# rrwick/Polypolish

Hardware: NVIDIA H100
Metric: assembly Mbp polished/sec (higher is better)
Workload: dtype u8 bases / u32 counters / f64 depth

## Files before the change

### polypolish_b200/csrc/polish_dev.cuh

```cuda
#pragma once

#include "nib_utils.h"
#include "../../include/pp_abi.h"

#define PP_BIN_SHIFT 8
#define PP_BIN (1u << PP_BIN_SHIFT)
#define PP_SUB_SHIFT 7
#define PP_SUB (1u << PP_SUB_SHIFT)
#define TL_T 2048
#define TL_THREADS 512
#define TL_PER_THREAD (TL_T / TL_THREADS)
#define TL_LONG_E 512
#define TL_QCAP 1024
#define TL_FAST_LEN 192
#define PR_THREADS 256
#define SC_GROUP_SCAN_LIMIT 8192
#define VT_THREADS 256
#define VT_ITEMS 8
#define VT_CHUNK (VT_THREADS * VT_ITEMS)
#define NONE32 0xFFFFFFFFu
static_assert(VT_CHUNK == TL_T, "k_tile hands k_compact one chunk per tile");
static_assert(TL_T % PP_BIN == 0 && TL_T / PP_SUB == TL_THREADS / 32 && TL_PER_THREAD * 32 == PP_SUB, "tile = whole bins; warp w owns depth sub-tile w and votes on it");

enum : unsigned {
// ... 1515 lines not shown
#endif
        __syncthreads();
        if (tid == 0) {
            long long t = 0;
            for (int i = 0; i < TL_THREADS / 32; ++i) t += sh.s_delta[i];
            vp.chunk_delta[tile] = t;
#ifdef PP_TILE_PROF
            pt[5] = clock64();
            for (int i = 0; i < 5; ++i) atomicAdd(&d.st->prof[i], (unsigned long long)(pt[i + 1] - pt[i]));
            atomicAdd(&d.st->prof[5], (unsigned long long)sh.qn);
            atomicAdd(&d.st->prof[6], 1ull);
            atomicMax(&d.st->prof[7], (unsigned long long)sh.qn);
#endif
        }
    }
}
static_assert(TL_PER_THREAD == 4, "the verdict store packs four positions per thread");

#if !defined(PP_EMULATE)
template <int BITS, bool CHG>
__global__ void __launch_bounds__(TL_THREADS, 1) k_tile(DevData d, VoteParams vp) {
    extern __shared__ __align__(16) unsigned char tile_smem[];
    tile_body<BITS, CHG>(d, vp, *reinterpret_cast<TileShared*>(tile_smem));
}
#endif

__device__ __forceinline__ uint8_t* put_u32(uint8_t* w, uint32_t v) {
    w[0] = (uint8_t)v; w[1] = (uint8_t)(v >> 8); w[2] = (uint8_t)(v >> 16); w[3] = (uint8_t)(v >> 24);
    return w + 4;
}
template <int BITS>
__device__ void allele_strings_row(const OthCtx& oc, uint32_t pos, uint32_t new_node, uint8_t* pool, unsigned long long cap,
                                   unsigned long long* used, unsigned long long* off) {
    unsigned long long bytes = 8;
    uint32_t n = 0;
    for (uint32_t nd = oc.head[pos]; nd != 0; nd = oc.nodes[nd - 1].next == NONE32 ? 0 : oc.nodes[nd - 1].next + 1) {
        bytes += 8 + ((uint32_t)oc.nodes[nd - 1].val & 0xFFFFu);
        n++;
    }
    const uint32_t new_len = new_node == NONE32 ? 0u : (uint32_t)oc.nodes[new_node].val & 0xFFFFu;
    bytes += new_len;
    const unsigned long long o = atomicAdd(used, bytes);
    *off = o;
    if (o + bytes > cap) return;
    uint8_t* w = put_u32(pool + o, n);
    for (uint32_t nd = oc.head[pos]; nd != 0; nd = oc.nodes[nd - 1].next == NONE32 ? 0 : oc.nodes[nd - 1].next + 1) {
        const uint32_t len = (uint32_t)oc.nodes[nd - 1].val & 0xFFFFu;
        w = put_u32(put_u32(w, oc.nodes[nd - 1].count), len);
        for (uint32_t t = 0; t < len; ++t) *w++ = other_char<BITS>(oc, nd - 1, t);
    }
    w = put_u32(w, new_len);
    for (uint32_t t = 0; t < new_len; ++t) *w++ = other_char<BITS>(oc, new_node, t);
}
template <int BITS>
__device__ void allele_strings_body(const OthCtx& oc, const uint32_t* pos, const pp_debug_pos* rec, bool by_pos, uint32_t n, uint8_t* pool,
                                    unsigned long long cap, unsigned long long* used, unsigned long long* off) {
    for (uint32_t i = blockIdx.x * blockDim.x + threadIdx.x; i < n; i += gridDim.x * blockDim.x) {
        const uint32_t p = pos[i];
        allele_strings_row<BITS>(oc, p, rec[by_pos ? p : i].new_node, pool, cap, used, off + i);
    }
}
#if !defined(PP_EMULATE)
template <int BITS>
__global__ void __launch_bounds__(256) k_allele_strings(OthCtx oc, const uint32_t* pos, const pp_debug_pos* rec, bool by_pos, uint32_t n,
                                                         uint8_t* pool, unsigned long long cap, unsigned long long* used, unsigned long long* off) {
    allele_strings_body<BITS>(oc, pos, rec, by_pos, n, pool, cap, used, off);
}
#endif

#define CP_STAGE (VT_CHUNK + 2048)
struct CompactShared {
    unsigned long long s_warp[VT_THREADS / 32];
    unsigned long long s_total;
    long long s_red[VT_THREADS / 32];
    long long s_base;
    __align__(16) uint8_t s_out[CP_STAGE];
};

template <int BITS>
__device__ __forceinline__ void compact_body(const DevData& d, const VoteParams& vp, CompactShared& sh) {
    const uint32_t tid = threadIdx.x, chunk = blockIdx.x;
    const uint32_t p0 = chunk * VT_CHUNK + tid * VT_ITEMS;
    long long acc = 0;
    for (uint32_t j = tid; j < chunk; j += VT_THREADS) acc += vp.chunk_delta[j];
    for (int o = 16; o > 0; o >>= 1) acc += __shfl_down_sync(0xffffffffu, acc, o);
    if ((tid & 31) == 0) sh.s_red[tid >> 5] = acc;
    __syncthreads();
    if (tid == 0) {
        long long t = 0;
        for (int i = 0; i < VT_THREADS / 32; ++i) t += sh.s_red[i];
        sh.s_base = (long long)chunk * VT_CHUNK + t;
    }
    const uint4 rv = *reinterpret_cast<const uint4*>(vp.res + p0);
    const uint32_t w[4] = {rv.x, rv.y, rv.z, rv.w};
    uint32_t len[VT_ITEMS];
    unsigned long long tlen = 0;
    OthCtx oc;
    oc.nodes = d.nodes; oc.head = d.oth_head;
    oc.sr = SeqRef{d.seq_pool, d.seq_off, d.seq_len, d.flags};
#pragma unroll
    for (int i = 0; i < VT_ITEMS; ++i) {
        const uint32_t h = (w[i >> 1] >> ((i & 1) * 16)) & 0xFFFFu;
        uint32_t l = h >> 8;
        if (p0 + i >= d.G) l = 0;
        else if (l == 255) {
            const uint32_t rec = vp.rec_at[p0 + i];
            const uint32_t rlen = (uint32_t)oc.nodes[rec].val & 0xFFFFu;
            l = 0;
            for (uint32_t t = 0; t < rlen; ++t) l += other_char<BITS>(oc, rec, t) != '-';
        }
        len[i] = l;
        tlen += l;
    }
    const unsigned long long oexcl = block_exscan<VT_THREADS>(tlen, sh.s_warp, &sh.s_total);
    const unsigned long long total = sh.s_total;
    const unsigned long long base = (unsigned long long)sh.s_base;
    if (chunk == vp.n_chunks - 1 && tid == 0) { vp.out_off[d.n_contigs] = base + total; d.st->out_len = base + total; }
    if (p0 < d.G) {
        uint32_t lo = 0, hi = d.n_contigs;
        while (lo < hi) { const uint32_t mid = (lo + hi) >> 1; if (d.contig_off[mid] < p0) lo = mid + 1; else hi = mid; }
        if (lo < d.n_contigs && d.contig_off[lo] < (unsigned long long)p0 + VT_ITEMS) {
            unsigned long long oo = base + oexcl;
            uint32_t c = lo;
#pragma unroll
            for (int i = 0; i < VT_ITEMS; ++i) {
                while (c < d.n_contigs && d.contig_off[c] == p0 + i) { vp.out_off[c] = oo; c++; }
                oo += len[i];
            }
        }
    }
    if (base + total > vp.out_cap) { if (tid == 0) atomicOr(&d.st->flags, (unsigned)FL_OUT_OVF); return; }
    const bool staged = total <= CP_STAGE;
    uint8_t* dst = staged ? sh.s_out : vp.out + base;
    unsigned long long o = oexcl;
#pragma unroll
    for (int i = 0; i < VT_ITEMS; ++i) {
        if (len[i] == 0) continue;
        const uint32_t h = (w[i >> 1] >> ((i & 1) * 16)) & 0xFFFFu;
        if ((h >> 8) != 255) { dst[o++] = (uint8_t)h; continue; }
        const uint32_t rec = vp.rec_at[p0 + i];
        const uint32_t rlen = (uint32_t)oc.nodes[rec].val & 0xFFFFu;
        for (uint32_t t = 0; t < rlen; ++t) {
            const uint8_t ch = other_char<BITS>(oc, rec, t);
            if (ch != '-') dst[o++] = ch;
        }
    }
    if (!staged) return;
    __syncthreads();
    uint8_t* g = vp.out + base;
    const uint32_t n = (uint32_t)total;
    const uint32_t head = min(n, (uint32_t)((16 - ((size_t)g & 15)) & 15));
    for (uint32_t i = tid; i < head; i += VT_THREADS) g[i] = sh.s_out[i];
    const uint32_t nvec = (n - head) / 16;
    for (uint32_t i = tid; i < nvec; i += VT_THREADS) {
        const uint8_t* sp = sh.s_out + head + i * 16;
        uint32_t x[4];
#pragma unroll
        for (int k = 0; k < 4; ++k) x[k] = sp[4 * k] | (sp[4 * k + 1] << 8) | (sp[4 * k + 2] << 16) | ((uint32_t)sp[4 * k + 3] << 24);
        reinterpret_cast<uint4*>(g + head)[i] = make_uint4(x[0], x[1], x[2], x[3]);
    }
    for (uint32_t i = head + nvec * 16 + tid; i < n; i += VT_THREADS) g[i] = sh.s_out[i];
}

#if !defined(PP_EMULATE)
template <int BITS>
__global__ void __launch_bounds__(VT_THREADS) k_compact(DevData d, VoteParams vp) {
    __shared__ CompactShared sh;
    compact_body<BITS>(d, vp, sh);
}
#endif
```

### polypolish_b200/csrc/polish_kernels.cu

```cuda
#include <cuda_runtime.h>

#include <cub/device/device_radix_sort.cuh>
#include <cub/device/device_scan.cuh>

#include <algorithm>
#include <functional>
#include <cstddef>
#include <cstdio>
#include <string>
#include <vector>

#include "pp_internal.h"
#include "pp_ctx.cuh"
#include "polish_dev.cuh"


static void init_comp_table(uint8_t* t) {
    for (int i = 0; i < 256; ++i) t[i] = 'N';
    const char* a = "ATGCNRYSWKMBVDH.-?";
    const char* b = "TACGNYRSWMKVBHD.-?";
    for (int i = 0; a[i]; ++i) t[(unsigned char)a[i]] = (uint8_t)b[i];
}

extern "C" const char* pp_version(void) { return "0.6.1-b200"; }

extern "C" void* pp_host_alloc(size_t bytes) {
    void* p = nullptr;
    if (cudaHostAlloc(&p, bytes ? bytes : 1, cudaHostAllocDefault) != cudaSuccess) { cudaGetLastError(); return nullptr; }
    return p;
}
extern "C" void pp_host_free(void* p) { if (p) cudaFreeHost(p); }

#define PP_INIT_IMAGE (64u << 10)

extern "C" int pp_create(int device, pp_ctx** out) {
    if (!out) return PP_ERR_ARG;
    *out = nullptr;
    int n = 0;
    cudaError_t e = cudaGetDeviceCount(&n);
    if (e != cudaSuccess || n == 0 || device < 0 || device >= n) { cudaGetLastError(); return PP_ERR_CUDA; }
    pp_ctx* ctx = new pp_ctx();
    ctx->device = device;
    if (cudaSetDevice(device) != cudaSuccess) { delete ctx; return PP_ERR_CUDA; }
    cudaDeviceProp prop;
    if (cudaGetDeviceProperties(&prop, device) != cudaSuccess || prop.major != 9 || prop.minor != 0) { delete ctx; return PP_ERR_CUDA; }
    ctx->sm_count = prop.multiProcessorCount;
    if (cudaStreamCreateWithFlags(&ctx->stream, cudaStreamNonBlocking) != cudaSuccess) { delete ctx; return PP_ERR_CUDA; }
    if (cudaStreamCreateWithFlags(&ctx->copy_stream, cudaStreamNonBlocking) != cudaSuccess) { delete ctx; return PP_ERR_CUDA; }
    if (cudaEventCreateWithFlags(&ctx->ev_small, cudaEventDisableTiming) != cudaSuccess ||
        cudaEventCreateWithFlags(&ctx->ev_seq, cudaEventDisableTiming) != cudaSuccess) { delete ctx; return PP_ERR_CUDA; }
    for (auto& ev : ctx->ev) if (cudaEventCreate(&ev) != cudaSuccess) { delete ctx; return PP_ERR_CUDA; }
    if (cudaHostAlloc((void**)&ctx->h_status, sizeof(DevStatus), cudaHostAllocDefault) != cudaSuccess) { delete ctx; return PP_ERR_CUDA; }
    if (cudaHostAlloc((void**)&ctx->h_params, sizeof(DevParams), cudaHostAllocDefault) != cudaSuccess) { delete ctx; return PP_ERR_CUDA; }
    if (cudaHostAlloc((void**)&ctx->h_init, PP_INIT_IMAGE, cudaHostAllocDefault) != cudaSuccess) { delete ctx; return PP_ERR_CUDA; }
    uint8_t comp[256];
    init_comp_table(comp);
    if (cudaMemcpyToSymbol(c_comp, comp, 256) != cudaSuccess) { delete ctx; return PP_ERR_CUDA; }
    *out = ctx;
    return PP_OK;
}

extern "C" void pp_destroy(pp_ctx* ctx) {
    if (!ctx) return;
    cudaSetDevice(ctx->device);
    if (ctx->stream) cudaStreamSynchronize(ctx->stream);
    pp_tok_release(ctx);
    for (auto& b : ctx->b) b.release();
    for (auto& ev : ctx->ev) if (ev) cudaEventDestroy(ev);
    if (ctx->h_status) cudaFreeHost(ctx->h_status);
    if (ctx->h_params) cudaFreeHost(ctx->h_params);
    if (ctx->h_init) cudaFreeHost(ctx->h_init);
    if (ctx->ev_small) cudaEventDestroy(ctx->ev_small);
    if (ctx->ev_seq) cudaEventDestroy(ctx->ev_seq);
    if (ctx->copy_stream) cudaStreamDestroy(ctx->copy_stream);
    if (ctx->stream) cudaStreamDestroy(ctx->stream);
    delete ctx;
}

extern "C" const char* pp_last_error(const pp_ctx* ctx) { return ctx ? ctx->err.c_str() : "null context"; }

int pp_ctx_fail(pp_ctx* ctx, int code, const char* msg) { ctx->err = msg; return code; }
int pp_ctx_device(pp_ctx* ctx) { return ctx->device; }
int pp_ctx_sm_count(pp_ctx* ctx) { return ctx->sm_count; }
cudaStream_t pp_ctx_stream(pp_ctx* ctx) { return ctx->stream; }
cudaEvent_t pp_ctx_event(pp_ctx* ctx, int i) { return ctx->ev[i]; }
void pp_ctx_count_launches(pp_ctx* ctx, uint32_t n) { ctx->launches = n; }
int pp_ctx_fail_cuda(pp_ctx* ctx, cudaError_t e, const char* what, const char* file, int line) {
    ctx->err = std::string("CUDA error: ") + cudaGetErrorString(e) + " at " + what + " (" + file + ":" + std::to_string(line) + ")";
    return PP_ERR_CUDA;
}
void* pp_ctx_scratch2(pp_ctx* ctx, size_t bytes) {
    if (ctx->b[B_SCRATCH2].ensure(bytes) != cudaSuccess) { cudaGetLastError(); return nullptr; }
    return ctx->b[B_SCRATCH2].p;
}
void* pp_ctx_scratch(pp_ctx* ctx, size_t bytes) {
    if (ctx->b[B_SCRATCH].ensure(bytes) != cudaSuccess) { cudaGetLastError(); return nullptr; }
    return ctx->b[B_SCRATCH].p;
}

template <class T>
static int upload(pp_ctx* ctx, int which, const T* src, size_t n, size_t pad_bytes = 64) {
    CK(ctx->b[which].ensure(n * sizeof(T) + pad_bytes));
    if (n) CK(cudaMemcpyAsync(ctx->b[which].p, src, n * sizeof(T), cudaMemcpyHostToDevice, ctx->stream));
    return PP_OK;
}

int pp_ctx_upload_contigs(pp_ctx* ctx, const pp_contigs* c) {
    if (!c || !c->off || !c->bases || c->n_contigs == 0) return ctx->fail(PP_ERR_ARG, "null or empty contigs");
    const uint64_t G = c->off[c->n_contigs];
    if (G == 0 || G >= 0xFFFFFFFFull - 2 * VT_CHUNK) return ctx->fail(PP_ERR_ARG, "total assembly length must be in [1, 2^32-4096)");
    int rc;
    if ((rc = upload(ctx, B_DRAFT, c->bases, G, VT_CHUNK + 256))) return rc;
    if ((rc = upload(ctx, B_CTGOFF, c->off, (size_t)c->n_contigs + 1))) return rc;
    ctx->G = G; ctx->n_contigs = c->n_contigs;
    return PP_OK;
}

static void fill_data(pp_ctx* ctx, DevData& d) {
    const uint64_t G = ctx->G;
    memset(&d, 0, sizeof d);
    d.n_aln = ctx->n_aln;
    d.contig = ctx->b[B_CONTIG].as<uint32_t>(); d.ref_start = ctx->b[B_REFSTART].as<uint32_t>();
    d.read_id = ctx->b[B_READID].as<uint32_t>(); d.seq_off = ctx->b[B_SEQOFF].as<uint32_t>();
    d.cigar_off = ctx->b[B_CIGOFF].as<uint32_t>(); d.nm = ctx->b[B_NM].as<uint32_t>();
    d.cigar_ops = ctx->b[B_CIGOPS].as<uint32_t>(); d.seq_len = ctx->b[B_SEQLEN].as<uint16_t>();
    d.n_cigar = ctx->b[B_NCIG].as<uint16_t>(); d.flags = ctx->b[B_FLAGS].as<uint8_t>();
    d.seq_pool = ctx->b[B_SEQPOOL].as<uint8_t>(); d.draft = ctx->b[B_DRAFT].as<uint8_t>();
    d.contig_off = ctx->b[B_CTGOFF].as<unsigned long long>(); d.n_contigs = ctx->n_contigs; d.G = (uint32_t)G;
    d.n_bins = (uint32_t)((G + PP_BIN - 1) >> PP_BIN_SHIFT); d.n_tiles = (uint32_t)((G + TL_T - 1) / TL_T);
    d.recs = ctx->b[B_RECS].as<TileRec>(); d.key = ctx->b[B_KEY].as<uint32_t>(); d.val = ctx->b[B_VAL].as<uint32_t>();
    d.sval = ctx->b[B_SVAL].as<uint32_t>(); d.bin_start = ctx->b[B_BINSTART].as<uint32_t>();
    d.srec = ctx->b[B_SREC].as<TileRec>(); d.sseq = ctx->b[B_SSEQ].as<uint4>();
    d.n_slots = ctx->n_slots; d.max_ext = ctx->max_ext;
    d.tile_order = ctx->b[B_TILEORDER].as<uint32_t>();
    d.kf = ctx->b[B_KF].as<uint32_t>(); d.wrec = ctx->b[B_NK].as<uint4>(); d.errc = ctx->b[B_ERRC].as<uint8_t>(); d.gq = ctx->b[B_GQ].as<uint16_t>();
}

template <int BITS>
static int bin_dataset(pp_ctx* ctx, const std::function<int()>& seq_ready) {
    cudaStream_t s = ctx->stream;
    const uint64_t n_aln = ctx->n_aln, G = ctx->G;
    const uint32_t n_bins = (uint32_t)((G + PP_BIN - 1) >> PP_BIN_SHIFT);
    int key_bits = 1;
    while ((1ull << key_bits) < (uint64_t)n_bins + 2) key_bits++;
    const size_t na = (size_t)n_aln + 16;
    CK(ctx->b[B_RECS].ensure(na * sizeof(TileRec)));
    CK(ctx->b[B_KEY].ensure(na * 4)); CK(ctx->b[B_VAL].ensure(na * 4));
    CK(ctx->b[B_SKEY].ensure(na * 4)); CK(ctx->b[B_SVAL].ensure(na * 4));
    CK(ctx->b[B_BINSTART].ensure(((size_t)n_bins + 4) * 4));
// ... 163 lines not shown
    const uint64_t seq_bytes = two_bit ? n_blocks2 * 16 + a->esc_pool_bytes : a->seq_pool_bytes;
    CK(ctx->b[B_SEQPOOL].ensure(seq_bytes + 256));
    if (two_bit) CK(ctx->b[B_SEQ2].ensure(a->seq_pool_bytes + 256));
    CK(cudaEventRecord(ctx->ev_small, ctx->stream));
    CK(cudaStreamWaitEvent(ctx->copy_stream, ctx->ev_small, 0));
    if (!two_bit) {
        if (a->seq_pool_bytes) CK(cudaMemcpyAsync(ctx->b[B_SEQPOOL].p, a->seq_pool, a->seq_pool_bytes, cudaMemcpyHostToDevice, ctx->copy_stream));
    } else {
        if (a->seq_pool_bytes) CK(cudaMemcpyAsync(ctx->b[B_SEQ2].p, a->seq_pool, a->seq_pool_bytes, cudaMemcpyHostToDevice, ctx->copy_stream));
        if (a->esc_pool_bytes)
            CK(cudaMemcpyAsync(ctx->b[B_SEQPOOL].as<uint8_t>() + n_blocks2 * 16, a->esc_pool, a->esc_pool_bytes, cudaMemcpyHostToDevice, ctx->copy_stream));
        if (a->esc_pool_bytes && a->n_aln)
            k_esc_offsets<<<(uint32_t)std::min<uint64_t>((a->n_aln + 255) / 256, (uint64_t)ctx->sm_count * 32), 256, 0, ctx->stream>>>(
                ctx->b[B_SEQOFF].as<uint32_t>(), ctx->b[B_FLAGS].as<uint8_t>(), a->n_aln, (uint32_t)n_blocks2);
    }
    CK(cudaEventRecord(ctx->ev_seq, ctx->copy_stream));
    auto seq_ready = [&]() -> int {
        CK(cudaStreamWaitEvent(ctx->stream, ctx->ev_seq, 0));
        if (two_bit && n_blocks2)
            k_expand2<<<(uint32_t)std::min<uint64_t>((n_blocks2 + 255) / 256, (uint64_t)ctx->sm_count * 32), 256, 0, ctx->stream>>>(
                ctx->b[B_SEQ2].as<uint2>(), ctx->b[B_SEQPOOL].as<uint4>(), n_blocks2);
        return PP_OK;
    };
    rc = commit_dataset(ctx, a->n_aln, a->n_reads, a->n_cigar_ops, seq_bytes, two_bit ? 4u : a->seq_bits, seq_ready);
    if (rc != PP_OK) cudaStreamSynchronize(ctx->copy_stream);
    return rc;
}

static const char* err_text(unsigned code) {
    switch (code) {
        case ERR_UNKNOWN_CONTIG: return "query name in SAM but not in assembly";
        case ERR_SEQ_MISMATCH: return "CIGAR string does not match read sequence";
        case ERR_BAD_OP: return "unexpected character (other than M, =, X, I or D) in CIGAR string - did you use BWA MEM to generate your alignments?";
        case ERR_OOB: return "alignment extends past the end of its reference sequence";
        case ERR_NOSEQ: return "no alignments for read contain sequence";
        default: return "unknown device-side error";
    }
}

template <int BITS>
static int run_polish(pp_ctx* ctx, const pp_polish_params* prm, pp_polish_result* res) {
    cudaStream_t s = ctx->stream;
    const uint64_t G = ctx->G, n_aln = ctx->n_aln;
    const uint32_t n_tiles = (uint32_t)((G + TL_T - 1) / TL_T);
    const size_t padG = (size_t)n_tiles * TL_T + 16;
    ctx->have_changes = false;

    CK(ctx->b[B_OUTOFF].ensure(((size_t)ctx->n_contigs + 1) * 8));
    CK(ctx->b[B_RES].ensure(padG * 2)); CK(ctx->b[B_RECAT].ensure((G + 1) * 4)); CK(ctx->b[B_CHUNKDELTA].ensure((size_t)n_tiles * 8));
    CK(ctx->b[B_PARAMS].ensure(sizeof(DevParams)));
    if (!ctx->tile_attr_set) {
        CK(cudaFuncSetAttribute(k_tile<4, false>, cudaFuncAttributeMaxDynamicSharedMemorySize, (int)sizeof(TileShared)));
        CK(cudaFuncSetAttribute(k_tile<8, false>, cudaFuncAttributeMaxDynamicSharedMemorySize, (int)sizeof(TileShared)));
        CK(cudaFuncSetAttribute(k_tile<4, true>, cudaFuncAttributeMaxDynamicSharedMemorySize, (int)sizeof(TileShared)));
        CK(cudaFuncSetAttribute(k_tile<8, true>, cudaFuncAttributeMaxDynamicSharedMemorySize, (int)sizeof(TileShared)));
        ctx->tile_attr_set = true;
    }

    ctx->h_params->fv = prm->fraction_valid; ctx->h_params->fi = prm->fraction_invalid;
    ctx->h_params->min_depth = prm->min_depth; ctx->h_params->max_errors = prm->max_errors;
    ctx->h_params->careful = prm->careful ? 1 : 0; ctx->h_params->pad = 0;

    for (int attempt = 0; attempt < 8; ++attempt) {
        const uint32_t node_cap = ctx->node_cap;
        const uint64_t out_cap = ctx->out_cap;
        size_t zoff = 0;
        auto carve = [&](size_t bytes) { size_t o = zoff; zoff += (bytes + 255) & ~size_t(255); return o; };
        const size_t o_chg = carve((size_t)ctx->n_contigs * 8), o_zero = carve((size_t)ctx->n_contigs * 8),
                     o_tdep = carve((size_t)ctx->n_contigs * 8), o_status = carve(sizeof(DevStatus)),
                     o_k = carve(ctx->global_k ? (ctx->n_reads + 1) * 4 : 4), o_prm = carve(sizeof(DevParams));
        const bool one_copy = zoff <= PP_INIT_IMAGE;
        CK(ctx->b[B_ZEROPOOL].ensure(zoff));
        CK(ctx->b[B_HEADS].ensure(padG * 4 + 64));
        uint8_t* zp = ctx->b[B_ZEROPOOL].as<uint8_t>();
        CK(ctx->b[B_NODES].ensure((size_t)node_cap * sizeof(OthNode)));
        CK(ctx->b[B_OUT].ensure(out_cap + 64));

        DevData d;
        fill_data(ctx, d);
        d.k = (uint32_t*)(zp + o_k);
        d.oth_head = ctx->b[B_HEADS].as<uint32_t>(); d.nodes = ctx->b[B_NODES].as<OthNode>(); d.node_cap = node_cap;
        d.prm = one_copy ? (DevParams*)(zp + o_prm) : ctx->b[B_PARAMS].as<DevParams>();
        d.st = (DevStatus*)(zp + o_status);
        ctx->launches = 0;

        CK(cudaEventRecord(ctx->ev[0], s));
        if (one_copy) {
            memset(ctx->h_init, 0, zoff);
            memcpy(ctx->h_init + o_prm, ctx->h_params, sizeof(DevParams));
            memset(ctx->h_init + o_status + offsetof(DevStatus, err), 0xFF, 8);
            CK(cudaMemcpyAsync(zp, ctx->h_init, zoff, cudaMemcpyHostToDevice, s));
        } else {
            CK(cudaMemcpyAsync(ctx->b[B_PARAMS].p, ctx->h_params, sizeof(DevParams), cudaMemcpyHostToDevice, s));
            CK(cudaMemsetAsync(zp, 0, zoff, s));
            CK(cudaMemsetAsync(&d.st->err, 0xFF, 8, s));
        }
        CK(cudaEventRecord(ctx->ev[1], s));
        if (n_aln && ctx->global_k) {
            k_classify_multi<<<(uint32_t)std::min<uint64_t>((n_aln + 255) / 256, (uint64_t)ctx->sm_count * 8), 256, 0, s>>>(d);
            ctx->launches++;
        }
        CK(cudaEventRecord(ctx->ev[2], s));
        if (n_aln) {
            const uint32_t grid = (uint32_t)std::min<uint64_t>((n_aln + PR_THREADS - 1) / PR_THREADS, (uint64_t)ctx->sm_count * 8);
            if (ctx->global_k) k_goodk<true><<<grid, PR_THREADS, 0, s>>>(d);
            else k_goodk<false><<<grid, PR_THREADS, 0, s>>>(d);
            ctx->launches++;
        }
        CK(cudaEventRecord(ctx->ev[3], s));
        VoteParams vp;
        vp.n_chunks = n_tiles;
        vp.out = ctx->b[B_OUT].as<uint8_t>(); vp.out_cap = out_cap;
        vp.out_off = ctx->b[B_OUTOFF].as<unsigned long long>();
        vp.changed = (unsigned long long*)(zp + o_chg); vp.zero_depth = (unsigned long long*)(zp + o_zero); vp.total_depth = (double*)(zp + o_tdep);
        vp.res = ctx->b[B_RES].as<uint16_t>(); vp.rec_at = ctx->b[B_RECAT].as<uint32_t>();
        vp.chunk_delta = ctx->b[B_CHUNKDELTA].as<long long>();
        vp.dbg = nullptr;
        if (ctx->debug_on) { CK(ctx->b[B_DEBUG].ensure((G + 1) * sizeof(pp_debug_pos))); vp.dbg = ctx->b[B_DEBUG].as<pp_debug_pos>(); }
        vp.chg = nullptr; vp.chg_pos = nullptr; vp.chg_n = &d.st->n_changes; vp.chg_cap = 0;
        if (ctx->changes_on) {
            if (ctx->chg_cap == 0) ctx->chg_cap = (uint32_t)std::max<uint64_t>(4096, G / 256);
            CK(ctx->b[B_CHG].ensure((size_t)ctx->chg_cap * sizeof(pp_debug_pos))); CK(ctx->b[B_CHGPOS].ensure((size_t)ctx->chg_cap * 4));
            vp.chg = ctx->b[B_CHG].as<pp_debug_pos>(); vp.chg_pos = ctx->b[B_CHGPOS].as<uint32_t>(); vp.chg_cap = ctx->chg_cap;
        }
        {
            int occ = 1;
            CK(cudaOccupancyMaxActiveBlocksPerMultiprocessor(&occ, vp.chg ? k_tile<BITS, true> : k_tile<BITS, false>, TL_THREADS, sizeof(TileShared)));
            const uint32_t grid = std::min<uint32_t>(n_tiles, (uint32_t)ctx->sm_count * (uint32_t)std::max(occ, 1));
            if (vp.chg) k_tile<BITS, true><<<grid, TL_THREADS, sizeof(TileShared), s>>>(d, vp);
            else k_tile<BITS, false><<<grid, TL_THREADS, sizeof(TileShared), s>>>(d, vp);
            ctx->launches++;
        }
        CK(cudaEventRecord(ctx->ev[4], s));
        k_compact<BITS><<<n_tiles, VT_THREADS, 0, s>>>(d, vp);
        ctx->launches++;
        CK(cudaEventRecord(ctx->ev[5], s));
        CK(cudaMemcpyAsync(ctx->h_status, d.st, sizeof(DevStatus), cudaMemcpyDeviceToHost, s));
        CK(cudaStreamSynchronize(s));
        CK(cudaGetLastError());
        const DevStatus hs = *ctx->h_status;
#ifdef PP_TILE_PROF
        fprintf(stderr, "[tile prof] tiles %llu; cycles/tile: A %.0f B %.0f queue %.0f C %.0f D+E %.0f; queued reads/tile %.1f (max %llu); "
                "chunk wait/tile/warp %.0f\n", hs.prof[6],
                (double)hs.prof[0] / hs.prof[6], (double)hs.prof[1] / hs.prof[6], (double)hs.prof[2] / hs.prof[6], (double)hs.prof[3] / hs.prof[6],
                (double)hs.prof[4] / hs.prof[6], (double)hs.prof[5] / hs.prof[6], hs.prof[7], (double)hs.prof[11] / hs.prof[6] / (TL_THREADS / 32));
        fprintf(stderr, "[tile prof] depth walks %llu (%.2f per tile, %llu tiles with one), %.0f cycles each\n", hs.prof[9], (double)hs.prof[9] / hs.prof[6], hs.prof[10],
                hs.prof[9] ? (double)hs.prof[8] / hs.prof[9] : 0.0);
#endif
        if (hs.err != ~0ull) {
            res->error_aln = (int64_t)(hs.err >> 8);
            return ctx->fail(PP_ERR_INPUT, std::string(err_text((unsigned)(hs.err & 0xFF))) + " (alignment " + std::to_string(hs.err >> 8) + ")");
        }
        bool again = false;
        if (hs.flags & FL_BIGGROUP) { if (ctx->global_k) return ctx->fail(PP_ERR_CUDA, "internal error: FL_BIGGROUP in global-k mode"); ctx->global_k = true; again = true; }
        if (hs.flags & FL_NODE_OVF) { ctx->node_cap = (uint32_t)std::min<uint64_t>(0x7FFFFFFFull, (uint64_t)hs.node_count + hs.node_count / 4 + 1024); again = true; }
        if (!again && (hs.flags & FL_OUT_OVF)) { ctx->out_cap = hs.out_len + 64; again = true; }
        if (!again && ctx->changes_on && hs.n_changes > ctx->chg_cap) { ctx->chg_cap = hs.n_changes; again = true; }
        if (again) continue;

        ctx->have_debug = ctx->debug_on; ctx->last_head = d.oth_head; ctx->last_nodes = std::min(hs.node_count, node_cap);
        ctx->have_changes = ctx->changes_on; ctx->n_changes = ctx->changes_on ? hs.n_changes : 0; ctx->chg_pool = -1;
        res->out_len = hs.out_len;
        res->n_aln_used = hs.n_used;
        res->error_aln = -1;
        memset(&res->timing, 0, sizeof res->timing);
        float ms;
        CK(cudaEventElapsedTime(&ms, ctx->ev[0], ctx->ev[1])); res->timing.stage_ms[0] = ms;
        CK(cudaEventElapsedTime(&ms, ctx->ev[1], ctx->ev[2])); res->timing.stage_ms[1] = ms;
        CK(cudaEventElapsedTime(&ms, ctx->ev[2], ctx->ev[3])); res->timing.stage_ms[2] = ms;
        CK(cudaEventElapsedTime(&ms, ctx->ev[3], ctx->ev[4])); res->timing.stage_ms[3] = ms;
        CK(cudaEventElapsedTime(&ms, ctx->ev[4], ctx->ev[5])); res->timing.stage_ms[4] = ms;
        CK(cudaEventElapsedTime(&ms, ctx->ev[0], ctx->ev[5])); res->timing.total_ms = ms;
        res->timing.launches = ctx->launches;

        if (res->out_bases) {
            if (res->out_cap < hs.out_len) return ctx->fail(PP_ERR_ARG, "out_cap too small: need " + std::to_string(hs.out_len) + " bytes");
            CK(cudaEventRecord(ctx->ev[7], s));
            CK(cudaMemcpyAsync(res->out_bases, vp.out, hs.out_len, cudaMemcpyDeviceToHost, s));
            if (res->out_off) CK(cudaMemcpyAsync(res->out_off, vp.out_off, ((size_t)ctx->n_contigs + 1) * 8, cudaMemcpyDeviceToHost, s));
            if (res->changed) CK(cudaMemcpyAsync(res->changed, vp.changed, (size_t)ctx->n_contigs * 8, cudaMemcpyDeviceToHost, s));
            if (res->zero_depth) CK(cudaMemcpyAsync(res->zero_depth, vp.zero_depth, (size_t)ctx->n_contigs * 8, cudaMemcpyDeviceToHost, s));
            if (res->total_depth) CK(cudaMemcpyAsync(res->total_depth, vp.total_depth, (size_t)ctx->n_contigs * 8, cudaMemcpyDeviceToHost, s));
            CK(cudaEventRecord(ctx->ev[8], s));
            CK(cudaStreamSynchronize(s));
            CK(cudaEventElapsedTime(&ms, ctx->ev[7], ctx->ev[8]));
            res->timing.stage_ms[7] = ms;
        }
        return PP_OK;
    }
    return ctx->fail(PP_ERR_NOMEM, "side buffers kept overflowing");
}

static int check_params(pp_ctx* ctx, const pp_polish_params* p) {
    if (!p) return ctx->fail(PP_ERR_ARG, "null params");
    if (!(p->fraction_valid > 0.0 && p->fraction_valid < 1.0)) return ctx->fail(PP_ERR_INPUT, "--fraction_valid must be between 0 and 1 (exclusive)");
    if (!(p->fraction_invalid > 0.0 && p->fraction_invalid < 1.0)) return ctx->fail(PP_ERR_INPUT, "--fraction_invalid must be between 0 and 1 (exclusive)");
    if (p->fraction_invalid >= p->fraction_valid) return ctx->fail(PP_ERR_INPUT, "--fraction_invalid must be less than --fraction_valid");
    return PP_OK;
}

extern "C" int pp_polish_resident(pp_ctx* ctx, const pp_polish_params* params, pp_polish_result* result) {
    if (!ctx) return PP_ERR_ARG;
    if (!result) return ctx->fail(PP_ERR_ARG, "null result");
    if (!ctx->have_ds) return ctx->fail(PP_ERR_ARG, "pp_polish_resident: no dataset uploaded");
    int rc = check_params(ctx, params);
    if (rc) return rc;
    CK(cudaSetDevice(ctx->device));
    result->error_aln = -1;
    return ctx->seq_bits == 4 ? run_polish<4>(ctx, params, result) : run_polish<8>(ctx, params, result);
}

extern "C" int pp_polish(pp_ctx* ctx, const pp_contigs* contigs, const pp_alignments* alns,
                         const pp_polish_params* params, pp_polish_result* result) {
    if (!ctx) return PP_ERR_ARG;
    if (!result) return ctx->fail(PP_ERR_ARG, "null result");
    int rc = check_params(ctx, params);
    if (rc) return rc;
    CK(cudaSetDevice(ctx->device));
    CK(cudaEventRecord(ctx->ev[9], ctx->stream));
    rc = pp_dataset_upload(ctx, contigs, alns);
    if (rc) return rc;
    CK(cudaEventRecord(ctx->ev[10], ctx->stream));
    CK(cudaEventSynchronize(ctx->ev[10]));
    float h2d = 0;
    CK(cudaEventElapsedTime(&h2d, ctx->ev[9], ctx->ev[10]));
    result->error_aln = -1;
    rc = ctx->seq_bits == 4 ? run_polish<4>(ctx, params, result) : run_polish<8>(ctx, params, result);
    if (rc == PP_OK) result->timing.stage_ms[6] = h2d;
    return rc;
}

extern "C" int pp_polish_set_debug(pp_ctx* ctx, int on) {
    if (!ctx) return PP_ERR_ARG;
    ctx->debug_on = on == 1;
    if (on == 0) ctx->have_debug = false;
    return PP_OK;
}

extern "C" int pp_polish_debug_fetch(pp_ctx* ctx, uint64_t first_pos, uint64_t n_pos, pp_debug_pos* out) {
    if (!ctx) return PP_ERR_ARG;
    if (!ctx->have_debug) return ctx->fail(PP_ERR_ARG, "pp_polish_debug_fetch: the last polish did not record debug positions (pp_polish_set_debug)");
    if (!out || first_pos + n_pos > ctx->G) return ctx->fail(PP_ERR_ARG, "pp_polish_debug_fetch: range outside the assembly");
    CK(cudaSetDevice(ctx->device));
    CK(cudaMemcpyAsync(out, ctx->b[B_DEBUG].as<pp_debug_pos>() + first_pos, n_pos * sizeof(pp_debug_pos), cudaMemcpyDeviceToHost, ctx->stream));
    CK(cudaStreamSynchronize(ctx->stream));
    return PP_OK;
}

extern "C" int pp_polish_debug_alleles(pp_ctx* ctx, uint32_t* head, pp_debug_node* nodes, uint64_t node_cap, uint64_t* n_nodes) {
    if (!ctx) return PP_ERR_ARG;
    if (!ctx->have_debug || !ctx->last_head) return ctx->fail(PP_ERR_ARG, "pp_polish_debug_alleles: no debug polish on this context");
    if (n_nodes) *n_nodes = ctx->last_nodes;
// ... 100 lines not shown
```

### polypolish_b200/csrc/pp_ctx.cuh

```cuda
#pragma once
#include <cuda_runtime.h>

#include <string>

#include "pp_internal.h"

struct DevStatus;
struct DevParams;
struct TokState;
struct pp_ctx;
void pp_tok_release(pp_ctx* ctx);

struct DevBuf {
    void* p = nullptr;
    size_t cap = 0;
    cudaError_t ensure(size_t bytes) {
        if (bytes <= cap) return cudaSuccess;
        if (p) cudaFree(p);
        p = nullptr; cap = 0;
        size_t want = bytes + bytes / 8 + 256;
        cudaError_t e = cudaMalloc(&p, want);
        if (e == cudaSuccess) cap = want;
        return e;
    }
    void release() { if (p) cudaFree(p); p = nullptr; cap = 0; }
    template <class T> T* as() const { return (T*)p; }
};

enum { B_CONTIG, B_REFSTART, B_READID, B_SEQOFF, B_SEQLEN, B_CIGOFF, B_NCIG, B_NM, B_FLAGS, B_CIGOPS, B_SEQPOOL,
       B_DRAFT, B_CTGOFF, B_ZEROPOOL, B_RECS, B_KEY, B_VAL, B_SKEY, B_SVAL, B_BINSTART, B_SREC, B_SSEQ, B_KF, B_NK, B_TILEORDER, B_ERRC, B_GQ, B_HEADS, B_NODES, B_CUBTMP, B_SEQ2, B_OUT,
       B_OUTOFF, B_DEBUG, B_RES, B_RECAT, B_CHUNKDELTA, B_PARAMS, B_SCRATCH, B_SCRATCH2,
       B_CHG, B_CHGPOS, B_STRPOS, B_STRPOOL, B_STROFF,
       B_TOKLINE, B_TOKTMP, B_TOKNAMES, B_COUNT };

struct pp_ctx {
    int device = 0;
    cudaStream_t stream = nullptr;
    cudaStream_t copy_stream = nullptr;
    cudaEvent_t ev_small = nullptr, ev_seq = nullptr;
    std::string err;
    DevBuf b[B_COUNT];
    cudaEvent_t ev[PP_N_STAGES + 4] = {};
    DevStatus* h_status = nullptr;
    DevParams* h_params = nullptr;
    uint8_t* h_init = nullptr;
    bool have_ds = false;
    uint64_t n_aln = 0, n_reads = 0, n_ops = 0, seq_bytes = 0, G = 0;
    uint32_t n_contigs = 0, seq_bits = 4;
    int sm_count = 132;
    uint32_t launches = 0;
    uint32_t node_cap = 0;
    uint32_t n_slots = 0, max_ext = 0;
    bool tile_attr_set = false;
    uint64_t out_cap = 0;
    bool global_k = false;
    bool debug_on = false, have_debug = false;
    const uint32_t* last_head = nullptr;
    uint32_t last_nodes = 0;
    bool changes_on = false, have_changes = false;
    uint32_t chg_cap = 0, n_changes = 0;
    int64_t chg_pool = -1;
    std::string changes_path;
    TokState* tok = nullptr;
    int parser = 0;

    int fail(int code, const std::string& m) { err = m; return code; }
    int fail_cuda(cudaError_t e, const char* what, const char* file, int line) {
        const char* base = file;
        for (const char* q = file; *q; ++q) if (*q == '/') base = q + 1;
        err = std::string("CUDA error: ") + cudaGetErrorString(e) + " at " + what + " (" + base + ":" + std::to_string(line) + ")";
        return PP_ERR_CUDA;
    }
};

#define CK(x) do { cudaError_t e_ = (x); if (e_ != cudaSuccess) return ctx->fail_cuda(e_, #x, __FILE__, __LINE__); } while (0)
```

Measured before the change: 8932.

## Capture polish kernel sequence into a cached CUDA graph and vectorize chunk-delta prefix sum

Captures the init copy/memset, classify, goodk, tile and compact launches into a CUDA graph keyed on the launch parameters, then replays it on later calls with the same key to cut per-launch host overhead. Events are recorded with the external flag so stage timing still works inside the graph. The compact kernel's prefix over chunk deltas now reads two 64-bit values per load with a 4-way unrolled loop, and its launch bounds request 8 blocks per SM. Risks: any buffer or parameter drift not captured in the key would replay stale pointers, and the host init image is refilled before launch because the captured memcpy reads it at replay time.

```diff
diff --git a/polypolish_b200/csrc/polish_dev.cuh b/polypolish_b200/csrc/polish_dev.cuh
--- a/polypolish_b200/csrc/polish_dev.cuh
+++ b/polypolish_b200/csrc/polish_dev.cuh
@@ -1621,7 +1621,16 @@
     const uint32_t tid = threadIdx.x, chunk = blockIdx.x;
     const uint32_t p0 = chunk * VT_CHUNK + tid * VT_ITEMS;
     long long acc = 0;
-    for (uint32_t j = tid; j < chunk; j += VT_THREADS) acc += vp.chunk_delta[j];
+    const ulonglong2* cd2 = reinterpret_cast<const ulonglong2*>(vp.chunk_delta);
+    const uint32_t pairs = chunk >> 1;
+    for (uint32_t j0 = tid; j0 < pairs; j0 += 4 * VT_THREADS) {
+        ulonglong2 v[4];
+#pragma unroll
+        for (int u = 0; u < 4; ++u) v[u] = j0 + u * VT_THREADS < pairs ? cd2[j0 + u * VT_THREADS] : make_ulonglong2(0, 0);
+#pragma unroll
+        for (int u = 0; u < 4; ++u) acc += (long long)(v[u].x + v[u].y);
+    }
+    if ((chunk & 1) && tid == 0) acc += vp.chunk_delta[chunk - 1];
     for (int o = 16; o > 0; o >>= 1) acc += __shfl_down_sync(0xffffffffu, acc, o);
     if ((tid & 31) == 0) sh.s_red[tid >> 5] = acc;
     __syncthreads();
@@ -1703,7 +1712,7 @@
 
 #if !defined(PP_EMULATE)
 template <int BITS>
-__global__ void __launch_bounds__(VT_THREADS) k_compact(DevData d, VoteParams vp) {
+__global__ void __launch_bounds__(VT_THREADS, 8) k_compact(DevData d, VoteParams vp) {
     __shared__ CompactShared sh;
     compact_body<BITS>(d, vp, sh);
 }
diff --git a/polypolish_b200/csrc/polish_kernels.cu b/polypolish_b200/csrc/polish_kernels.cu
--- a/polypolish_b200/csrc/polish_kernels.cu
+++ b/polypolish_b200/csrc/polish_kernels.cu
@@ -65,6 +65,7 @@
     cudaSetDevice(ctx->device);
     if (ctx->stream) cudaStreamSynchronize(ctx->stream);
     pp_tok_release(ctx);
+    if (ctx->polish_graph) cudaGraphExecDestroy(ctx->polish_graph);
     for (auto& b : ctx->b) b.release();
     for (auto& ev : ctx->ev) if (ev) cudaEventDestroy(ev);
     if (ctx->h_status) cudaFreeHost(ctx->h_status);
@@ -394,33 +395,8 @@
         d.oth_head = ctx->b[B_HEADS].as<uint32_t>(); d.nodes = ctx->b[B_NODES].as<OthNode>(); d.node_cap = node_cap;
         d.prm = one_copy ? (DevParams*)(zp + o_prm) : ctx->b[B_PARAMS].as<DevParams>();
         d.st = (DevStatus*)(zp + o_status);
-        ctx->launches = 0;
-
-        CK(cudaEventRecord(ctx->ev[0], s));
-        if (one_copy) {
-            memset(ctx->h_init, 0, zoff);
-            memcpy(ctx->h_init + o_prm, ctx->h_params, sizeof(DevParams));
-            memset(ctx->h_init + o_status + offsetof(DevStatus, err), 0xFF, 8);
-            CK(cudaMemcpyAsync(zp, ctx->h_init, zoff, cudaMemcpyHostToDevice, s));
-        } else {
-            CK(cudaMemcpyAsync(ctx->b[B_PARAMS].p, ctx->h_params, sizeof(DevParams), cudaMemcpyHostToDevice, s));
-            CK(cudaMemsetAsync(zp, 0, zoff, s));
-            CK(cudaMemsetAsync(&d.st->err, 0xFF, 8, s));
-        }
-        CK(cudaEventRecord(ctx->ev[1], s));
-        if (n_aln && ctx->global_k) {
-            k_classify_multi<<<(uint32_t)std::min<uint64_t>((n_aln + 255) / 256, (uint64_t)ctx->sm_count * 8), 256, 0, s>>>(d);
-            ctx->launches++;
-        }
-        CK(cudaEventRecord(ctx->ev[2], s));
-        if (n_aln) {
-            const uint32_t grid = (uint32_t)std::min<uint64_t>((n_aln + PR_THREADS - 1) / PR_THREADS, (uint64_t)ctx->sm_count * 8);
-            if (ctx->global_k) k_goodk<true><<<grid, PR_THREADS, 0, s>>>(d);
-            else k_goodk<false><<<grid, PR_THREADS, 0, s>>>(d);
-            ctx->launches++;
-        }
-        CK(cudaEventRecord(ctx->ev[3], s));
         VoteParams vp;
+        memset(&vp, 0, sizeof vp);
         vp.n_chunks = n_tiles;
         vp.out = ctx->b[B_OUT].as<uint8_t>(); vp.out_cap = out_cap;
         vp.out_off = ctx->b[B_OUTOFF].as<unsigned long long>();
@@ -435,18 +411,77 @@
             CK(ctx->b[B_CHG].ensure((size_t)ctx->chg_cap * sizeof(pp_debug_pos))); CK(ctx->b[B_CHGPOS].ensure((size_t)ctx->chg_cap * 4));
             vp.chg = ctx->b[B_CHG].as<pp_debug_pos>(); vp.chg_pos = ctx->b[B_CHGPOS].as<uint32_t>(); vp.chg_cap = ctx->chg_cap;
         }
+        const bool classify = n_aln && ctx->global_k;
+        const uint32_t grid_classify = (uint32_t)std::min<uint64_t>((n_aln + 255) / 256, (uint64_t)ctx->sm_count * 8);
+        const uint32_t grid_goodk = (uint32_t)std::min<uint64_t>((n_aln + PR_THREADS - 1) / PR_THREADS, (uint64_t)ctx->sm_count * 8);
+        uint32_t grid_tile;
         {
             int occ = 1;
             CK(cudaOccupancyMaxActiveBlocksPerMultiprocessor(&occ, vp.chg ? k_tile<BITS, true> : k_tile<BITS, false>, TL_THREADS, sizeof(TileShared)));
-            const uint32_t grid = std::min<uint32_t>(n_tiles, (uint32_t)ctx->sm_count * (uint32_t)std::max(occ, 1));
-            if (vp.chg) k_tile<BITS, true><<<grid, TL_THREADS, sizeof(TileShared), s>>>(d, vp);
-            else k_tile<BITS, false><<<grid, TL_THREADS, sizeof(TileShared), s>>>(d, vp);
-            ctx->launches++;
-        }
-        CK(cudaEventRecord(ctx->ev[4], s));
-        k_compact<BITS><<<n_tiles, VT_THREADS, 0, s>>>(d, vp);
-        ctx->launches++;
-        CK(cudaEventRecord(ctx->ev[5], s));
+            grid_tile = std::min<uint32_t>(n_tiles, (uint32_t)ctx->sm_count * (uint32_t)std::max(occ, 1));
+        }
+        cudaEvent_t ev_goodk = classify ? ctx->ev[2] : ctx->ev[1];
+
+        auto enqueue = [&]() -> cudaError_t {
+            cudaError_t e;
+            auto mark = [&](cudaEvent_t ev) { return cudaEventRecordWithFlags(ev, s, cudaEventRecordExternal); };
+            if ((e = mark(ctx->ev[0]))) return e;
+            if (one_copy) {
+                if ((e = cudaMemcpyAsync(zp, ctx->h_init, zoff, cudaMemcpyHostToDevice, s))) return e;
+            } else {
+                if ((e = cudaMemcpyAsync(ctx->b[B_PARAMS].p, ctx->h_params, sizeof(DevParams), cudaMemcpyHostToDevice, s))) return e;
+                if ((e = cudaMemsetAsync(zp, 0, zoff, s))) return e;
+                if ((e = cudaMemsetAsync(&d.st->err, 0xFF, 8, s))) return e;
+            }
+            if ((e = mark(ctx->ev[1]))) return e;
+            if (classify) {
+                k_classify_multi<<<grid_classify, 256, 0, s>>>(d);
+                if ((e = mark(ev_goodk))) return e;
+            }
+            if (n_aln) {
+                if (ctx->global_k) k_goodk<true><<<grid_goodk, PR_THREADS, 0, s>>>(d);
+                else k_goodk<false><<<grid_goodk, PR_THREADS, 0, s>>>(d);
+            }
+            if ((e = mark(ctx->ev[3]))) return e;
+            if (vp.chg) k_tile<BITS, true><<<grid_tile, TL_THREADS, sizeof(TileShared), s>>>(d, vp);
+            else k_tile<BITS, false><<<grid_tile, TL_THREADS, sizeof(TileShared), s>>>(d, vp);
+            if ((e = mark(ctx->ev[4]))) return e;
+            k_compact<BITS><<<n_tiles, VT_THREADS, 0, s>>>(d, vp);
+            if ((e = mark(ctx->ev[5]))) return e;
+            return cudaGetLastError();
+        };
+        ctx->launches = (classify ? 1u : 0u) + (n_aln ? 1u : 0u) + 2u;
+
+        struct Key { DevData d; VoteParams vp; uint32_t grid_classify, grid_goodk, grid_tile, bits; uint64_t zoff; uint32_t one_copy, classify; };
+        Key key;
+        memset(&key, 0, sizeof key);
+        memcpy(&key.d, &d, sizeof d); memcpy(&key.vp, &vp, sizeof vp);
+        key.grid_classify = grid_classify; key.grid_goodk = grid_goodk; key.grid_tile = grid_tile; key.bits = BITS;
+        key.zoff = zoff; key.one_copy = one_copy; key.classify = classify;
+        if (!ctx->polish_graph || ctx->polish_key.size() != sizeof key || memcmp(ctx->polish_key.data(), &key, sizeof key) != 0) {
+            if (ctx->polish_graph) { cudaGraphExecDestroy(ctx->polish_graph); ctx->polish_graph = nullptr; }
+            CK(cudaStreamBeginCapture(s, cudaStreamCaptureModeThreadLocal));
+            const cudaError_t ee = enqueue();
+            cudaGraph_t g = nullptr;
+            const cudaError_t ec = cudaStreamEndCapture(s, &g);
+            if (ee != cudaSuccess || ec != cudaSuccess) {
+                if (g) cudaGraphDestroy(g);
+                cudaGetLastError();
+                return ctx->fail_cuda(ee != cudaSuccess ? ee : ec, "capturing the polish call", __FILE__, __LINE__);
+            }
+            cudaGraphExec_t ge = nullptr;
+            const cudaError_t ei = cudaGraphInstantiate(&ge, g, 0);
+            cudaGraphDestroy(g);
+            CK(ei);
+            ctx->polish_graph = ge;
+            ctx->polish_key.assign(reinterpret_cast<const char*>(&key), sizeof key);
+        }
+        if (one_copy) {
+            memset(ctx->h_init, 0, zoff);
+            memcpy(ctx->h_init + o_prm, ctx->h_params, sizeof(DevParams));
+            memset(ctx->h_init + o_status + offsetof(DevStatus, err), 0xFF, 8);
+        }
+        CK(cudaGraphLaunch(ctx->polish_graph, s));
         CK(cudaMemcpyAsync(ctx->h_status, d.st, sizeof(DevStatus), cudaMemcpyDeviceToHost, s));
         CK(cudaStreamSynchronize(s));
         CK(cudaGetLastError());
@@ -478,8 +513,8 @@
         memset(&res->timing, 0, sizeof res->timing);
         float ms;
         CK(cudaEventElapsedTime(&ms, ctx->ev[0], ctx->ev[1])); res->timing.stage_ms[0] = ms;
-        CK(cudaEventElapsedTime(&ms, ctx->ev[1], ctx->ev[2])); res->timing.stage_ms[1] = ms;
-        CK(cudaEventElapsedTime(&ms, ctx->ev[2], ctx->ev[3])); res->timing.stage_ms[2] = ms;
+        CK(cudaEventElapsedTime(&ms, ctx->ev[1], ev_goodk)); res->timing.stage_ms[1] = ms;
+        CK(cudaEventElapsedTime(&ms, ev_goodk, ctx->ev[3])); res->timing.stage_ms[2] = ms;
         CK(cudaEventElapsedTime(&ms, ctx->ev[3], ctx->ev[4])); res->timing.stage_ms[3] = ms;
         CK(cudaEventElapsedTime(&ms, ctx->ev[4], ctx->ev[5])); res->timing.stage_ms[4] = ms;
         CK(cudaEventElapsedTime(&ms, ctx->ev[0], ctx->ev[5])); res->timing.total_ms = ms;
diff --git a/polypolish_b200/csrc/pp_ctx.cuh b/polypolish_b200/csrc/pp_ctx.cuh
--- a/polypolish_b200/csrc/pp_ctx.cuh
+++ b/polypolish_b200/csrc/pp_ctx.cuh
@@ -52,6 +52,8 @@
     uint32_t node_cap = 0;
     uint32_t n_slots = 0, max_ext = 0;
     bool tile_attr_set = false;
+    cudaGraphExec_t polish_graph = nullptr;
+    std::string polish_key;
     uint64_t out_cap = 0;
     bool global_k = false;
     bool debug_on = false, have_debug = false;
```

After: 9049, median of 6. 1.01x the previous value.
